# JuliaDiffusionBayes/DiffusionMCMCTools.jl

Measured on NVIDIA B200. Metric: guided path updates/sec (chains x EM steps/s, FP64), higher is better.
Workload: dtype f64

## Files before the change

diffusionmcmctools.jl_b200/csrc/dmt_api.cu:

```cuda
#include "../../include/dmt.h"
#include "kernels.cuh"
#include "fwd_kernel.cuh"
#include "sweep_kernel.cuh"
#include "sweep_ws_kernel.cuh"
#include "sweep_sp_kernel.cuh"
#include "tsit5_kernel.cuh"
#include "moments_kernel.cuh"

#include <algorithm>
#include <atomic>
#include <nvtx3/nvToolsExt.h>
#include <cmath>
#include <cstdio>
#include <cstring>
#include <dlfcn.h>
#include <stdexcept>
#include <string>
#include <unordered_map>
#include <vector>

using namespace dmt;

#ifdef DMT_ONLY_MODEL
#define DMT_FOR_MODELS(X) X(DMT_ONLY_MODEL)
#else
#define DMT_FOR_MODELS(X) X(M_FHN) X(M_LV) X(M_LORENZ) X(M_PROK) X(M_JR) X(M_OU2)
#endif

namespace {

struct DmtError : std::runtime_error {
    int code;
    DmtError(int c, const std::string &m) : std::runtime_error(m), code(c) {}
};

#define CK(call)                                                                                                   \
    do {                                                                                                           \
        cudaError_t e_ = (call);                                                                                   \
        if (e_ != cudaSuccess)                                                                                     \
            throw DmtError(DMT_ERR_CUDA, std::string(#call) + ": " + cudaGetErrorString(e_));                      \
    } while (0)
#define REQUIRE(cond, code, msg)                                                                                   \
    do {                                                                                                           \
        if (!(cond)) throw DmtError(code, msg);                                                                    \
    } while (0)

std::string g_create_error;
std::atomic<unsigned long long> g_launches{0};

struct ModelDims { int D, DW, NPAR; bool constdiff; };
bool model_dims(int model, ModelDims &md) {
    switch (model) {
    case M_FHN: md = {Model<M_FHN>::D, Model<M_FHN>::DW, Model<M_FHN>::NPAR, Model<M_FHN>::CONSTDIFF}; return true;
    case M_LV: md = {Model<M_LV>::D, Model<M_LV>::DW, Model<M_LV>::NPAR, Model<M_LV>::CONSTDIFF}; return true;
    case M_LORENZ: md = {Model<M_LORENZ>::D, Model<M_LORENZ>::DW, Model<M_LORENZ>::NPAR, Model<M_LORENZ>::CONSTDIFF}; return true;
    case M_PROK: md = {Model<M_PROK>::D, Model<M_PROK>::DW, Model<M_PROK>::NPAR, Model<M_PROK>::CONSTDIFF}; return true;
    case M_JR: md = {Model<M_JR>::D, Model<M_JR>::DW, Model<M_JR>::NPAR, Model<M_JR>::CONSTDIFF}; return true;
    case M_OU2: md = {Model<M_OU2>::D, Model<M_OU2>::DW, Model<M_OU2>::NPAR, Model<M_OU2>::CONSTDIFF}; return true;
    }
    return false;
}

template <class T> struct DevBuf {
    T *p = nullptr;
    size_t n = 0;
    void alloc(size_t count, bool zero = true) {
        release();
        n = count;
        if (count) {
            CK(cudaMalloc(&p, count * sizeof(T)));
            if (zero) {
                CK(cudaMemsetAsync(p, 0, count * sizeof(T), cudaStreamLegacy));
                CK(cudaStreamSynchronize(cudaStreamLegacy));
            }
        }
    }
    void release() {
        if (p) cudaFree(p);
        p = nullptr;
        n = 0;
    }
    ~DevBuf() { release(); }
    DevBuf() = default;
    DevBuf(const DevBuf &) = delete;
    DevBuf &operator=(const DevBuf &) = delete;
    DevBuf(DevBuf &&o) noexcept : p(o.p), n(o.n) { o.p = nullptr; o.n = 0; }
};

struct Layout {
    bool set = false;
    int nb = 0;
    std::vector<int> i0, i1;
    std::vector<uint8_t> last;
    DevBuf<int> d_i0, d_i1;
    DevBuf<uint8_t> d_last, d_ok, d_last_acc, d_acc_hist;
    DevBuf<double> d_rho, d_ll, d_ll_hist;
    LayoutDev dev{};
    bool cache_enabled = false, cache_valid = false;
    bool F_stale = false;
    DevBuf<double> d_Gl[2], d_c0l[2], d_FP[2], d_cq, d_vlast;
    DevBuf<int> d_blk_of_k;
};

struct NcclApi {
    void *h = nullptr;
    int (*GetUniqueId)(void *) = nullptr;
    int (*CommInitRank)(void **, int, struct UidByValue, int) = nullptr;
    int (*AllReduce)(const void *, void *, size_t, int, int, void *, cudaStream_t) = nullptr;
    int (*CommDestroy)(void *) = nullptr;
    const char *(*GetErrorString)(int) = nullptr;
};
struct UidByValue { char internal[128]; };
NcclApi g_nccl;
void load_nccl() {
    if (g_nccl.h) return;
    const char *names[] = {"libnccl.so.2", "libnccl.so"};
    for (const char *nm : names) {
        g_nccl.h = dlopen(nm, RTLD_NOW | RTLD_GLOBAL);
        if (g_nccl.h) break;
    }
    REQUIRE(g_nccl.h, DMT_ERR_NCCL, std::string("dlopen(libnccl.so.2) failed: ") + dlerror());
    g_nccl.GetUniqueId = (int (*)(void *))dlsym(g_nccl.h, "ncclGetUniqueId");
    g_nccl.CommInitRank = (int (*)(void **, int, UidByValue, int))dlsym(g_nccl.h, "ncclCommInitRank");
    g_nccl.AllReduce = (int (*)(const void *, void *, size_t, int, int, void *, cudaStream_t))dlsym(g_nccl.h, "ncclAllReduce");
    g_nccl.CommDestroy = (int (*)(void *))dlsym(g_nccl.h, "ncclCommDestroy");
    g_nccl.GetErrorString = (const char *(*)(int))dlsym(g_nccl.h, "ncclGetErrorString");
    REQUIRE(g_nccl.GetUniqueId && g_nccl.CommInitRank && g_nccl.AllReduce && g_nccl.CommDestroy, DMT_ERR_NCCL, "NCCL symbols missing");
}
#define NCK(call)                                                                                                  \
    do {                                                                                                           \
        int r_ = (call);                                                                                           \
        if (r_ != 0)                                                                                               \
            throw DmtError(DMT_ERR_NCCL, std::string(#call) + ": " + (g_nccl.GetErrorString ? g_nccl.GetErrorString(r_) : "nccl error")); \
    } while (0)

}

struct dmt_ctx {
    dmt_config cfg{};
    ModelDims md{};
    int D = 0, DW = 0, NPAR = 0, NH = 0, NG = 0, NAUX = 0, NOBS = 0;
    int K = 0, M = 0, P = 0, m = 0, NT = 0, NTb = 0, S = 0, NP = 0;
    std::vector<int> nsteps, tile0, step0, pt0, ppb_tile0;
    cudaStream_t stream = nullptr;
    DevCtx dev{};
    std::vector<Layout> layouts;
    std::string err;
    DevBuf<int> d_tile0, d_step0, d_pt0, d_nsteps, d_ppb_tile0, d_pset, d_k_of_tile, d_k_of_ppbtile;
    DevBuf<double> d_dt, d_sqdt, d_X, d_W, d_X0;
    DevBuf<uint8_t> d_parX, d_parW, d_parP[2];
    DevBuf<double> d_G[2][2], d_c0[2][2], d_theta[2][2], d_aux[2][2], d_obs[2], d_vart[2];
    DevBuf<double> d_scratch, d_partial, d_stats;
    DevBuf<uint8_t> d_mask;
    DevBuf<int> d_flag;
    void *nccl_comm = nullptr;
    P2PBuf *p2p_local = nullptr;
    P2PArgs p2p{};
    bool p2p_ready = false;
    int n_ranks = 1;
    int fwd_lanes = 0;
    int bwd_solver = 0;
    double bwd_reltol = 1e-3, bwd_abstol = 1e-6;
    DevBuf<int> d_steps;
    int bwd_mode = 0;
    DevBuf<double> d_xbar[2];
    std::vector<char> xbar_set[2];
    cudaStream_t copy_stream = nullptr;
    cudaEvent_t ev_gathered = nullptr, ev_copied = nullptr, ev_hist = nullptr;
    DevBuf<double> d_snap;
    DevBuf<int> d_snap_sel;
    bool pipe_ok = false;
    int sweep_mode = 0;
    std::unordered_map<const void *, size_t> resident;
    bool lazy_W = false;
    char last_fwd_kernel[96] = "";
    int W_stale_layout = -1;
    int G_owner = -1;
    bool parP_mixed = false;
    bool aux_all_linearised = true;
    DevBuf<double> d_pm_mean, d_pm_m2;
    uint64_t pm_count = 0;
    DevBuf<int> d_pm_cs, d_pm_chains;

    double *scratch(size_t n) {
        if (d_scratch.n < n) d_scratch.alloc(n, false);
        return d_scratch.p;
    }
};

namespace {

Layout &layout_of(dmt_ctx *c, int id) {
    REQUIRE(id >= 0 && id < (int)c->layouts.size(), DMT_ERR_ARG, "layout index out of range");
    REQUIRE(c->layouts[id].set, DMT_ERR_STATE, "layout not registered (dmt_set_blocks)");
    return c->layouts[id];
}

void check_side(dmt_ctx *c, int side) {
    REQUIRE(side == 0 || side == 1, DMT_ERR_ARG, "side must be 0 (accepted) or 1 (proposal)");
}
void check_law_side(dmt_ctx *c, int side) {
    check_side(c, side);
    REQUIRE(side == 0 || c->cfg.two_sided_laws, DMT_ERR_STATE, "proposal laws not allocated (dmt_config.two_sided_laws = 0)");
}
void check_range(dmt_ctx *c, int k0, int k1) { REQUIRE(0 <= k0 && k0 <= k1 && k1 < c->K, DMT_ERR_ARG, "interval range out of bounds"); }

dim3 chain_grid(dmt_ctx *c, int ny, int tpb) { return dim3((c->M + tpb - 1) / tpb, ny, 1); }
dim3 pset_grid(dmt_ctx *c, int ny, int tpb, int nz = 1) { return dim3((c->P + tpb - 1) / tpb, ny, nz); }

template <class Kernel> size_t resident_ctas(dmt_ctx *c, Kernel *kernel, int threads, size_t smem) {
    const auto it = c->resident.find((const void *)kernel);
    if (it != c->resident.end()) return it->second;
    int per_sm = 0, sms = 0;
    CK(cudaFuncSetAttribute(kernel, cudaFuncAttributeMaxDynamicSharedMemorySize, (int)smem));
    CK(cudaOccupancyMaxActiveBlocksPerMultiprocessor(&per_sm, kernel, threads, smem));
    CK(cudaDeviceGetAttribute(&sms, cudaDevAttrMultiProcessorCount, c->cfg.device));
    return c->resident[(const void *)kernel] = (size_t)per_sm * sms;
}

template <int OP> constexpr bool fwd_coop() { return OP == OP_DRAW || OP == OP_INIT || OP == OP_SWEEP; }
template <class MD> constexpr int fwd_tpb() { return MD::D >= 6 ? 32 : FWD_TPB; }
template <class MD, int OP, int G> size_t fwd_wave_threads(dmt_ctx *c) {
    return resident_ctas(c, fwd_kernel<MD, OP, fwd_tpb<MD>(), G>, fwd_tpb<MD>(), 0) * fwd_tpb<MD>();
}
template <class MD, int OP, int G> void launch_fwd_g(dmt_ctx *c, Layout &L, const FwdArgs &fa) {
    constexpr int TPB = fwd_tpb<MD>();
    fwd_wave_threads<MD, OP, G>(c);
    const dim3 grid((unsigned)(((size_t)c->M * G + TPB - 1) / TPB), L.nb, 1);
    snprintf(c->last_fwd_kernel, sizeof(c->last_fwd_kernel), "fwd_kernel<op=%d, lanes=%d%s>", OP, G, (OP == OP_SWEEP && fa.lazy_w) ? ", lazy" : "");
    ++g_launches, fwd_kernel<MD, OP, TPB, G><<<grid, TPB, 0, c->stream>>>(c->dev, L.dev, fa);
}
template <class MD, int OP> void launch_fwd_tile(dmt_ctx *c, Layout &L, const FwdArgs &fa, int lanes) {
    if constexpr (fwd_coop<OP>()) {
        if (lanes == 8) return launch_fwd_g<MD, OP, 8>(c, L, fa);
        if (lanes == 4) return launch_fwd_g<MD, OP, 4>(c, L, fa);
        if (lanes == 2) return launch_fwd_g<MD, OP, 2>(c, L, fa);
    }
    launch_fwd_g<MD, OP, 1>(c, L, fa);
}
template <class MD, int OP> int tile_lanes(dmt_ctx *c, const Layout &L) {
    if constexpr (fwd_coop<OP>()) {
        if (c->fwd_lanes) return c->fwd_lanes;
        if (MD::DW < 2) return 1;
        const size_t units = (size_t)c->M * L.nb;
        if (OP != OP_SWEEP) {
            if (units * 8 <= fwd_wave_threads<MD, OP, 8>(c)) return 8;
            if (units * 4 <= fwd_wave_threads<MD, OP, 4>(c)) return 4;
        }
        if (units * 2 <= fwd_wave_threads<MD, OP, 2>(c)) return 2;
    }
    return 1;
}

void ensure_guiding(dmt_ctx *c, Layout &L);
void ensure_W(dmt_ctx *c);
bool covers_all_intervals(dmt_ctx *c, const Layout &L) {
    std::vector<char> seen(c->K, 0);
    for (int b = 0; b < L.nb; b++)
        for (int k = L.i0[b]; k <= L.i1[b]; k++) seen[k] = 1;
    return std::all_of(seen.begin(), seen.end(), [](char s) { return s != 0; });
}

template <class MD, bool LAZY> void launch_sweep_pipe(dmt_ctx *c, Layout &L, const FwdArgs &fa) {
    constexpr size_t smem = sweep_pipe_smem<MD>();
    resident_ctas(c, sweep_pipe_kernel<MD, LAZY>, 32, smem);
    const dim3 grid((unsigned)((c->M + 31) / 32), L.nb, 1);
    snprintf(c->last_fwd_kernel, sizeof(c->last_fwd_kernel), "sweep_pipe_kernel<lanes=1%s>", LAZY ? ", lazy" : "");
    ++g_launches, sweep_pipe_kernel<MD, LAZY><<<grid, 32, smem, c->stream>>>(c->dev, L.dev, fa);
}
template <class MD> using WsWide = WsShape<6, (MD::D <= 3 ? 8 : MD::D == 4 ? 6 : 3), (MD::D <= 3 ? 4 : MD::D == 4 ? 3 : 2)>;
template <class MD, bool LAZY> size_t ws_resident_ctas(dmt_ctx *c) {
    constexpr size_t smem = sweep_ws_smem<MD, WsWide<MD>>();
    static_assert(smem <= 227 * 1024, "the rings of the warp-specialised sweep must fit one SM's shared memory");
    return resident_ctas(c, sweep_ws_kernel<MD, LAZY, WsWide<MD>>, WsWide<MD>::THREADS, smem);
}
template <class MD, bool LAZY> void launch_sweep_ws(dmt_ctx *c, Layout &L, const FwdArgs &fa) {
    using SH = WsWide<MD>;
    ws_resident_ctas<MD, LAZY>(c);
    const dim3 grid((unsigned)((c->M + 31) / 32), L.nb, 1);
    snprintf(c->last_fwd_kernel, sizeof(c->last_fwd_kernel), "sweep_ws_kernel<wide, %s>", LAZY ? "lazy" : "eager");
    ++g_launches, sweep_ws_kernel<MD, LAZY, SH><<<grid, SH::THREADS, sweep_ws_smem<MD, SH>(), c->stream>>>(c->dev, L.dev, fa);
}
template <class MD, bool LAZY> void launch_sweep_sp(dmt_ctx *c, Layout &L, const FwdArgs &fa) {
    const dim3 grid((unsigned)((c->M + 7) / 8), L.nb, 1);
    snprintf(c->last_fwd_kernel, sizeof(c->last_fwd_kernel), "sweep_sp_kernel<step lanes=4%s>", LAZY ? ", lazy" : "");
    ++g_launches, sweep_sp_kernel<MD, LAZY><<<grid, 32, 0, c->stream>>>(c->dev, L.dev, fa);
}

struct SweepChoice {
    enum Kernel { TILE, PIPE, WS, SP } kernel;
    int lanes;
    bool lazy;
};
template <class MD> SweepChoice pick_sweep(dmt_ctx *c, const Layout &L, const FwdArgs &fa) {
    const bool lazy = c->lazy_W && !fa.Z && covers_all_intervals(c, L);
    const bool eligible = c->pipe_ok && !c->parP_mixed && !fa.Z && fa.skip == 0;
    const int mode = c->sweep_mode;
    if (mode >= 2) {
        REQUIRE(eligible, DMT_ERR_UNSUPPORTED, "pipelined sweep needs one parameter set per chain in chain order, uniform law parity and device RNG");
        if (mode == 3) return {SweepChoice::WS, 1, lazy};
        if (mode == 5) return {SweepChoice::SP, 1, lazy};
        REQUIRE(c->fwd_lanes <= 1, DMT_ERR_UNSUPPORTED, "the pipelined sweep maps one lane to a (chain, block)");
        return {SweepChoice::PIPE, 1, lazy};
    }
    const SweepChoice tile{SweepChoice::TILE, tile_lanes<MD, OP_SWEEP>(c, L), lazy};
    if (mode == 1 || !eligible || c->fwd_lanes) return tile;
    const size_t ws_units = (size_t)((c->M + 31) / 32) * L.nb;
    if (ws_units <= (lazy ? ws_resident_ctas<MD, true>(c) : ws_resident_ctas<MD, false>(c))) return {SweepChoice::WS, 1, lazy};
    if (MD::DW >= 2 && (size_t)c->M * L.nb <= 14080) return {SweepChoice::SP, 1, lazy};
    if (tile.lanes == 2 || !lazy) return tile;
    return {SweepChoice::PIPE, 1, lazy};
}

template <class MD, int OP> void launch_fwd_model(dmt_ctx *c, Layout &L, FwdArgs fa) {
    if constexpr (OP == OP_SWEEP) {
        const SweepChoice s = pick_sweep<MD>(c, L, fa);
        fa.lazy_w = s.lazy;
        switch (s.kernel) {
        case SweepChoice::TILE: launch_fwd_tile<MD, OP>(c, L, fa, s.lanes); break;
        case SweepChoice::PIPE: s.lazy ? launch_sweep_pipe<MD, true>(c, L, fa) : launch_sweep_pipe<MD, false>(c, L, fa); break;
        case SweepChoice::WS: s.lazy ? launch_sweep_ws<MD, true>(c, L, fa) : launch_sweep_ws<MD, false>(c, L, fa); break;
        case SweepChoice::SP: s.lazy ? launch_sweep_sp<MD, true>(c, L, fa) : launch_sweep_sp<MD, false>(c, L, fa); break;
        }
        if (s.lazy) c->W_stale_layout = L.dev.id;
    } else {
        launch_fwd_tile<MD, OP>(c, L, fa, tile_lanes<MD, OP>(c, L));
    }
}

template <int OP> void launch_fwd(dmt_ctx *c, Layout &L, const FwdArgs &fa) {
    if (c->W_stale_layout >= 0 && OP != OP_LOGLIK) {
        const bool rewrites_all = (OP == OP_INIT) || ((OP == OP_INVSOLVE || OP == OP_INVSOLVE_LL || OP == OP_SWEEP) && covers_all_intervals(c, L));
        if (rewrites_all) c->W_stale_layout = -1;
        else ensure_W(c);
    }
    ensure_guiding(c, L);
#define DMT_CASE(MID)                                                                                              \
    case MID: launch_fwd_model<Model<MID>, OP>(c, L, fa); break;
    switch (c->cfg.model) {
        DMT_FOR_MODELS(DMT_CASE)
        default: throw DmtError(DMT_ERR_UNSUPPORTED, "model not compiled into this build of libdmt");
    }
#undef DMT_CASE
    CK(cudaGetLastError());
}

template <class MD> void launch_bwd_model(dmt_ctx *c, Layout &L, const BwdArgs &ba) {
    const int nz = c->cfg.two_sided_laws ? 2 : 1;
    if (c->bwd_solver == 1) {
        REQUIRE(!ba.use_override, DMT_ERR_UNSUPPORTED, "the guiding cache needs the RK4 backward filter (its F is affine in v only there)");
        if (c->d_steps.n < 2) c->d_steps.alloc(2);
// ... 482 lines not shown
        dim3 grid = pset_grid(ctx, k1 - k0 + 1, 128);
#define DMT_CASE(MID)                                                                                              \
    case MID: ++g_launches, aux_linearise_kernel<Model<MID>><<<grid, 128, 0, ctx->stream>>>(ctx->dev, side, store, k0, k1, tmp); break;
        switch (ctx->cfg.model) {
            DMT_FOR_MODELS(DMT_CASE)
        default: throw DmtError(DMT_ERR_UNSUPPORTED, "model not compiled into this build of libdmt");
        }
#undef DMT_CASE
        CK(cudaGetLastError());
        CK(cudaStreamSynchronize(ctx->stream));
    });
}

int32_t dmt_set_obs(dmt_ctx *ctx, int32_t side, int32_t k0, int32_t k1, const double *L, const double *Sigma, const double *v) {
    return guarded(ctx, [&] {
        check_law_side(ctx, side); check_range(ctx, k0, k1);
        if (side == 0) { ensure_W(ctx); invalidate_caches(ctx); }
        REQUIRE(L && Sigma && v, DMT_ERR_ARG, "null observation array");
        const int m = ctx->m, D = ctx->D;
        double *r0 = ctx->d_obs[0].p, *r1 = ctx->d_obs[1].p;
        put_record(ctx, side, 0, r0, r1, ctx->NOBS, 0, m * D, k0, k1, L, false);
        put_record(ctx, side, 0, r0, r1, ctx->NOBS, m * D, m * m, k0, k1, Sigma, false);
        put_record(ctx, side, 0, r0, r1, ctx->NOBS, m * D + m * m, m, k0, k1, v, false);
    });
}

int32_t dmt_equalize_laws(dmt_ctx *ctx, int32_t store_mask, int32_t k0, int32_t k1, int32_t *changed) {
    return guarded(ctx, [&] {
        check_law_side(ctx, 1); check_range(ctx, k0, k1);
        dim3 grid = pset_grid(ctx, k1 - k0 + 1, 128);
        if (ctx->d_flag.n < 1) ctx->d_flag.alloc(1);
        CK(cudaMemsetAsync(ctx->d_flag.p, 0, sizeof(int), ctx->stream));
        for (int st = 0; st < 2; st++) {
            if (!((store_mask >> st) & 1)) continue;
            ++g_launches, copy_record_kernel<<<grid, 128, 0, ctx->stream>>>(ctx->dev, st, ctx->d_theta[0][st].p, ctx->d_theta[1][st].p, ctx->NPAR, k0, k1, ctx->d_flag.p);
            ++g_launches, copy_record_kernel<<<grid, 128, 0, ctx->stream>>>(ctx->dev, st, ctx->d_aux[0][st].p, ctx->d_aux[1][st].p, ctx->NAUX, k0, k1, ctx->d_flag.p);
            if (st == 0) ++g_launches, copy_record_kernel<<<grid, 128, 0, ctx->stream>>>(ctx->dev, 0, ctx->d_obs[0].p, ctx->d_obs[1].p, ctx->NOBS, k0, k1, ctx->d_flag.p);
        }
        CK(cudaGetLastError());
        if (changed) {
            int h = 0;
            CK(cudaMemcpyAsync(&h, ctx->d_flag.p, sizeof(int), cudaMemcpyDeviceToHost, ctx->stream));
            CK(cudaStreamSynchronize(ctx->stream));
            *changed = h;
        }
    });
}

int32_t dmt_set_blocks(dmt_ctx *ctx, int32_t layout, int32_t n_blocks, const int32_t *i0, const int32_t *i1, const double *rho,
                       const uint8_t *last, int32_t ll_hist_len) {
    return guarded(ctx, [&] {
        REQUIRE(layout >= 0 && layout < (int)ctx->layouts.size(), DMT_ERR_ARG, "layout index out of range");
        REQUIRE(n_blocks >= 1 && n_blocks <= 64 && i0 && i1 && rho, DMT_ERR_ARG, "need 1 <= n_blocks <= 64 and non-null ranges/rho");
        Layout &L = ctx->layouts[layout];
        std::vector<uint8_t> lst(n_blocks);
        for (int b = 0; b < n_blocks; b++) {
            lst[b] = last ? (last[b] ? 1 : 0) : (b == n_blocks - 1 ? 1 : 0);
            REQUIRE(0 <= i0[b] && i0[b] <= i1[b] && i1[b] < ctx->K, DMT_ERR_ARG, "block range out of bounds");
            REQUIRE(lst[b] || i1[b] > i0[b], DMT_ERR_ARG, "a non-terminal block must span at least 2 intervals");
            REQUIRE(lst[b] || ctx->P == ctx->M, DMT_ERR_UNSUPPORTED,
                    "blocking freezes a per-recording artificial observation: needs n_psets == n_chains");
            REQUIRE(std::abs(rho[b]) <= 1.0, DMT_ERR_ARG, "rho must be in [-1, 1]");
        }
        const size_t M = ctx->M;
        L.nb = n_blocks;
        L.i0.assign(i0, i0 + n_blocks); L.i1.assign(i1, i1 + n_blocks); L.last = lst;
        L.d_i0.alloc(n_blocks); L.d_i1.alloc(n_blocks); L.d_last.alloc(n_blocks); L.d_rho.alloc(n_blocks);
        L.d_ll.alloc(2 * n_blocks * M); L.d_ok.alloc(n_blocks * M); L.d_last_acc.alloc(n_blocks * M);
        CK(cudaMemcpy(L.d_i0.p, i0, sizeof(int) * n_blocks, cudaMemcpyHostToDevice));
        CK(cudaMemcpy(L.d_i1.p, i1, sizeof(int) * n_blocks, cudaMemcpyHostToDevice));
        CK(cudaMemcpy(L.d_last.p, lst.data(), n_blocks, cudaMemcpyHostToDevice));
        CK(cudaMemcpy(L.d_rho.p, rho, sizeof(double) * n_blocks, cudaMemcpyHostToDevice));
        {
            std::vector<double> ninf(2 * n_blocks * M, -INFINITY);
            CK(cudaMemcpy(L.d_ll.p, ninf.data(), sizeof(double) * ninf.size(), cudaMemcpyHostToDevice));
        }
        const int hl_req = ll_hist_len >= 0 ? ll_hist_len : ctx->cfg.ll_hist_len;
        const size_t hl = hl_req > 0 ? hl_req : 0;
        if (hl) { L.d_acc_hist.alloc(hl * n_blocks * M); L.d_ll_hist.alloc(hl * 2 * n_blocks * M); }
        L.dev.nb = n_blocks; L.dev.id = layout;
        L.dev.i0 = L.d_i0.p; L.dev.i1 = L.d_i1.p; L.dev.last = L.d_last.p; L.dev.rho = L.d_rho.p;
        L.dev.ll = L.d_ll.p; L.dev.ok = L.d_ok.p; L.dev.last_acc = L.d_last_acc.p;
        L.dev.acc_hist = hl ? L.d_acc_hist.p : nullptr; L.dev.ll_hist = hl ? L.d_ll_hist.p : nullptr; L.dev.hist_len = (int)hl;
        L.set = true;
        L.cache_enabled = false; L.cache_valid = false;
        cache_set_private(L, false);
        rebuild_ppb_store(ctx);
    });
}

int32_t dmt_set_rho(dmt_ctx *ctx, int32_t layout, const double *rho) {
    return guarded(ctx, [&] {
        Layout &L = layout_of(ctx, layout);
        REQUIRE(rho, DMT_ERR_ARG, "null rho");
        CK(cudaMemcpyAsync(L.d_rho.p, rho, sizeof(double) * L.nb, cudaMemcpyHostToDevice, ctx->stream));
        CK(cudaStreamSynchronize(ctx->stream));
    });
}

int32_t dmt_set_start(dmt_ctx *ctx, const double *x0) {
    return guarded(ctx, [&] {
        REQUIRE(x0, DMT_ERR_ARG, "null x0");
        const size_t n = (size_t)ctx->D * ctx->M;
        for (int s = 0; s < 2; s++)
            CK(cudaMemcpyAsync(ctx->d_X0.p + s * ctx->dev.X0buf, x0, n * sizeof(double), cudaMemcpyHostToDevice, ctx->stream));
        CK(cudaStreamSynchronize(ctx->stream));
    });
}

static void xfer_paths(dmt_ctx *ctx, int side, double *host, bool is_x, bool upload) {
    check_side(ctx, side);
    REQUIRE(host, DMT_ERR_ARG, "null host array");
    if (!is_x) {
        if (upload && side == 0) ctx->W_stale_layout = -1;
        else ensure_W(ctx);
    }
    const size_t n = is_x ? (size_t)ctx->NP * ctx->D * ctx->M : (size_t)ctx->S * ctx->DW * ctx->M;
    DevBuf<double> nat;
    nat.alloc(n, false);
    if (upload) CK(cudaMemcpyAsync(nat.p, host, n * sizeof(double), cudaMemcpyHostToDevice, ctx->stream));
    dim3 grid = chain_grid(ctx, ctx->K, 128);
    if (is_x) ++g_launches, xfer_X_kernel<<<grid, 128, 0, ctx->stream>>>(ctx->dev, side, ctx->D, nat.p, upload ? 1 : 0);
    else ++g_launches, xfer_W_kernel<<<grid, 128, 0, ctx->stream>>>(ctx->dev, side, ctx->DW, nat.p, upload ? 1 : 0);
    CK(cudaGetLastError());
    if (!upload) CK(cudaMemcpyAsync(host, nat.p, n * sizeof(double), cudaMemcpyDeviceToHost, ctx->stream));
    CK(cudaStreamSynchronize(ctx->stream));
}
int32_t dmt_set_X(dmt_ctx *ctx, int32_t side, const double *X) { return guarded(ctx, [&] { xfer_paths(ctx, side, (double *)X, true, true); }); }
int32_t dmt_get_X(dmt_ctx *ctx, int32_t side, double *X) { return guarded(ctx, [&] { xfer_paths(ctx, side, X, true, false); }); }
int32_t dmt_set_W(dmt_ctx *ctx, int32_t side, const double *W) { return guarded(ctx, [&] { xfer_paths(ctx, side, (double *)W, false, true); }); }
int32_t dmt_get_W(dmt_ctx *ctx, int32_t side, double *W) { return guarded(ctx, [&] { xfer_paths(ctx, side, W, false, false); }); }

int32_t dmt_snapshot_paths_async(dmt_ctx *ctx, int32_t side, int32_t n_sel, const int32_t *chains, double *host_out) {
    return guarded(ctx, [&] {
        check_side(ctx, side);
        REQUIRE(n_sel >= 1 && chains && host_out, DMT_ERR_ARG, "bad snapshot arguments");
        for (int i = 0; i < n_sel; i++) REQUIRE(chains[i] >= 0 && chains[i] < ctx->M, DMT_ERR_ARG, "chain index out of range");
        if (!ctx->copy_stream) {
            CK(cudaStreamCreateWithFlags(&ctx->copy_stream, cudaStreamNonBlocking));
            CK(cudaEventCreateWithFlags(&ctx->ev_gathered, cudaEventDisableTiming));
            CK(cudaEventCreateWithFlags(&ctx->ev_copied, cudaEventDisableTiming));
            CK(cudaEventRecord(ctx->ev_copied, ctx->copy_stream));
        }
        const size_t n = (size_t)ctx->NP * ctx->D * n_sel;
        CK(cudaStreamWaitEvent(ctx->stream, ctx->ev_copied, 0));
        if (ctx->d_snap.n < n) { CK(cudaStreamSynchronize(ctx->copy_stream)); ctx->d_snap.alloc(n, false); }
        if (ctx->d_snap_sel.n < (size_t)n_sel) { CK(cudaStreamSynchronize(ctx->copy_stream)); ctx->d_snap_sel.alloc(n_sel, false); }
        CK(cudaMemcpyAsync(ctx->d_snap_sel.p, chains, sizeof(int) * n_sel, cudaMemcpyHostToDevice, ctx->stream));
        ++g_launches, gather_X_kernel<<<dim3((n_sel + 63) / 64, ctx->K), 64, 0, ctx->stream>>>(ctx->dev, side, ctx->D, ctx->d_snap_sel.p, n_sel, ctx->d_snap.p);
        CK(cudaGetLastError());
        CK(cudaEventRecord(ctx->ev_gathered, ctx->stream));
        CK(cudaStreamWaitEvent(ctx->copy_stream, ctx->ev_gathered, 0));
        CK(cudaMemcpyAsync(host_out, ctx->d_snap.p, n * sizeof(double), cudaMemcpyDeviceToHost, ctx->copy_stream));
        CK(cudaEventRecord(ctx->ev_copied, ctx->copy_stream));
    });
}
static void get_paths_of(dmt_ctx *ctx, int side, int n_sel, const int32_t *chains, double *out, bool is_x) {
    check_side(ctx, side);
    if (!is_x) ensure_W(ctx);
    REQUIRE(n_sel >= 1 && chains && out, DMT_ERR_ARG, "bad chain selection");
    for (int i = 0; i < n_sel; i++) REQUIRE(chains[i] >= 0 && chains[i] < ctx->M, DMT_ERR_ARG, "chain index out of range");
    const size_t n = (is_x ? (size_t)ctx->NP * ctx->D : (size_t)ctx->S * ctx->DW) * n_sel;
    DevBuf<double> d;
    DevBuf<int> sel;
    d.alloc(n, false);
    sel.alloc(n_sel, false);
// ... 682 lines not shown
```

diffusionmcmctools.jl_b200/csrc/sweep_kernel.cuh:

```cuda
#pragma once
#include "fwd_kernel.cuh"
#include <type_traits>

namespace dmt {

template <int N, int I = 0, class F> __device__ __forceinline__ void static_for(F &&f) {
    if constexpr (I < N) {
        f(std::integral_constant<int, I>{});
        static_for<N, I + 1>(f);
    }
}

__device__ __forceinline__ bool elect_one_lane() {
    uint32_t pred;
    asm volatile("{\n.reg .pred p;\nelect.sync _|p, 0xffffffff;\nselp.u32 %0, 1, 0, p;\n}" : "=r"(pred));
    return pred != 0;
}
template <class MD> constexpr int sweep_pipe_minb() { return MD::D <= 3 ? 10 : 1; }

template <class MD> constexpr size_t sweep_pipe_smem() {
    constexpr int D = MD::D, NG = D * (D + 1) / 2 + D;
    return (size_t)2 * (NG * 128 + 8) * 8 + (size_t)(D * D + D) * 32 * 8 + 2 * 8;
}

template <class MD, bool LAZYW>
__global__ void __launch_bounds__(32, sweep_pipe_minb<MD>()) sweep_pipe_kernel(const DevCtx cx, const LayoutDev ly, const FwdArgs fa) {
    constexpr int D = MD::D, DW = MD::DW, NPAR = MD::NPAR, NH = D * (D + 1) / 2, NG = NH + D, NAUX = D * D + D + NH;
    constexpr int STAGE = NG * 128 + 8;
    extern __shared__ __align__(128) unsigned char sw_smem[];
    double *ring = reinterpret_cast<double *>(sw_smem);
    double *cst = ring + 2 * STAGE;
    uint64_t *bars = reinterpret_cast<uint64_t *>(cst + (D * D + D) * 32);

    const int lane = threadIdx.x;
    const int c0 = blockIdx.x * 32, b = blockIdx.y;
    if (c0 >= cx.M) return;
    const int c_raw = c0 + lane;
    const int c = min(c_raw, cx.M - 1);
    const bool live = c_raw < cx.M;
    const size_t M = cx.M, P = cx.P;
    const int ps = c;
    const int i0 = ly.i0[b], i1 = ly.i1[b];
    const bool last = ly.last[b] != 0;
    const double rho = ly.rho[b], crho = sqrt(1.0 - rho * rho);
    const uint32_t chunk_bytes = 32u * (uint32_t)min(32, cx.M - c0);
    const size_t gstr = P * 4;

    if (lane == 0) { mbar_init(&bars[0], 1); mbar_init(&bars[1], 1); }
    asm volatile("fence.mbarrier_init.release.cluster;" ::: "memory");
    __syncwarp();

    int kn = i0, qn = 0, ntl_n = (cx.nsteps[i0] + 3) >> 2, t0_n = cx.tile0[i0], n_prod = 0;
    const double *gp_n = g_tile_of<NG>(cx, ly, i0, i1, last, 0, c0).base;
    const double *xin_n = cx.X + (size_t)cx.parX[(size_t)i0 * M + c] * cx.Xbuf + ((size_t)t0_n * D * M + c) * 4;
    bool more = true;
    double xnx[D][4];
    auto prefetch = [&]() {
        if (!more) return;
        if (elect_one_lane()) {
            uint64_t *bar = &bars[n_prod & 1];
            double *dst = ring + (size_t)(n_prod & 1) * STAGE;
            mbar_expect_tx(bar, NG * chunk_bytes + 64u);
#pragma unroll
            for (int a = 0; a < NG; a++) bulk_g2s(dst + a * 128, gp_n + ((size_t)qn * NG + a) * gstr, chunk_bytes, bar);
            bulk_g2s(dst + NG * 128, cx.dt + (size_t)(t0_n + qn) * 4, 32u, bar);
            bulk_g2s(dst + NG * 128 + 4, cx.sqdt + (size_t)(t0_n + qn) * 4, 32u, bar);
        }
#pragma unroll
        for (int i = 0; i < D; i++) ld256(xin_n + ((size_t)qn * D + i) * M * 4, xnx[i]);
        n_prod++;
        if (++qn == ntl_n) {
            qn = 0;
            if (++kn <= i1) {
                ntl_n = (cx.nsteps[kn] + 3) >> 2;
                t0_n = cx.tile0[kn];
                gp_n = g_tile_of<NG>(cx, ly, kn, i1, last, 0, c0).base;
                xin_n = cx.X + (size_t)cx.parX[(size_t)kn * M + c] * cx.Xbuf + ((size_t)t0_n * D * M + c) * 4;
            } else more = false;
        }
    };
    prefetch();

    double x[D], xo[D];
    {
        const int sl = cx.parX[(size_t)i0 * M + c];
#pragma unroll
        for (int i = 0; i < D; i++) { x[i] = cx.X0[sl * cx.X0buf + ((size_t)i0 * D + i) * M + c]; xo[i] = x[i]; }
    }
    double ll = 0.0, llo = 0.0;
    bool ok = true;
    int n_cons = 0;

    for (int k = i0; k <= i1; ++k) {
        const GTile<NG> gt = g_tile_of<NG>(cx, ly, k, i1, last, 0, ps);
        double th[NPAR];
        {
            const double *tp = cx.theta[gt.slot][gt.store] + (size_t)k * NPAR * P + ps;
#pragma unroll
            for (int i = 0; i < NPAR; i++) th[i] = tp[(size_t)i * P];
        }
        const typename MD::Par par(th);
        {
            const double *ap = cx.aux[gt.slot][gt.store] + (size_t)k * NAUX * P + ps;
#pragma unroll
            for (int i = 0; i < D * D + D; i++) cst[i * 32 + lane] = ap[(size_t)i * P];
        }
        double at[NH];
        if (!MD::CONSTDIFF) {
            const double *ap = cx.aux[gt.slot][gt.store] + (size_t)k * NAUX * P + ps;
#pragma unroll
            for (int i = 0; i < NH; i++) at[i] = ap[(size_t)(D * D + D + i) * P];
        }
        const int nst = cx.nsteps[k], t0 = cx.tile0[k];
        const uint8_t pw = cx.parW[(size_t)k * M + c], px = cx.parX[(size_t)k * M + c];
        double *Wacc = cx.W + (size_t)pw * cx.Wbuf + ((size_t)t0 * DW * M + c) * 4;
        double *Wprop = cx.W + (size_t)(1 ^ pw) * cx.Wbuf + ((size_t)t0 * DW * M + c) * 4;
        double *Xout = cx.X + (size_t)(1 ^ px) * cx.Xbuf + ((size_t)t0 * D * M + c) * 4;
        if (k > i0) {
#pragma unroll
            for (int i = 0; i < D; i++) x[i] = cx.X0[(size_t)px * cx.X0buf + ((size_t)k * D + i) * M + c];
        }
        if (live) {
            double *x0p = cx.X0 + (size_t)(1 ^ px) * cx.X0buf + (size_t)k * D * M + c;
#pragma unroll
            for (int i = 0; i < D; i++) x0p[(size_t)i * M] = xo[i];
        }
        const int ntl = (nst + 3) >> 2;
        for (int q = 0; q < ntl; ++q) {
            double xt[D][4];
#pragma unroll
            for (int i = 0; i < D; i++)
#pragma unroll
                for (int s = 0; s < 4; s++) xt[i][s] = xnx[i][s];
            prefetch();
            if (q == ntl - 1 && k < i1) {
                const int k1 = k + 1;
                const int store1 = (k1 == i1 && !last) ? 1 : 0;
                const int slot1 = cx.parP[store1][(size_t)k1 * P + ps];
                const double *tp = cx.theta[slot1][store1] + (size_t)k1 * NPAR * P + ps;
#pragma unroll
                for (int i = 0; i < NPAR; i++) prefetch_l2(tp + (size_t)i * P);
                const double *ap = cx.aux[slot1][store1] + (size_t)k1 * NAUX * P + ps;
#pragma unroll
                for (int i = 0; i < (MD::CONSTDIFF ? D * D + D : NAUX); i++) prefetch_l2(ap + (size_t)i * P);
#pragma unroll
                for (int i = 0; i < D; i++) {
                    prefetch_l2(cx.X0 + ((size_t)k1 * D + i) * M + c);
                    prefetch_l2(cx.X0 + cx.X0buf + ((size_t)k1 * D + i) * M + c);
                }
                prefetch_l2(cx.parX + (size_t)k1 * M + c);
                prefetch_l2(cx.parW + (size_t)k1 * M + c);
            }
            double z[4 * DW];
            tile_normals<DW>(cx.seed, cx.chain_offset + (uint32_t)c, (uint32_t)(t0 + q), fa.iter, (uint32_t)ly.id, z);

            mbar_wait(&bars[n_cons & 1], (uint32_t)(n_cons >> 1) & 1u);
            const double *st = ring + (size_t)(n_cons & 1) * STAGE;
            const double *sg = st + lane * 4;
            n_cons++;
            if (k == i0 && q == 0) {
                double s0 = -*gt.c0;
#pragma unroll
                for (int i = 0; i < D; i++) {
                    double hx = 0.0;
#pragma unroll
                    for (int j = 0; j < D; j++) hx = fma(sg[sidx<D>(i, j) * 128], x[j], hx);
                    s0 += x[i] * (sg[(NH + i) * 128] - 0.5 * hx);
                }
                ll = s0;
                llo = s0;
            }
            double w[LAZYW ? 1 : DW][4], wo[LAZYW ? 1 : DW][4], xot[D][4];
            auto step = [&](auto s_c, auto full_c) {
                constexpr int s = decltype(s_c)::value;
                constexpr bool FULL = decltype(full_c)::value;
                const int i = 4 * q + s;
                if (FULL || i < nst) {
                    double Hs[NH], F[D], Bm[D * D], beta[D], gd[D], G = 0.0;
#pragma unroll
                    for (int a = 0; a < NH; a++) Hs[a] = sg[a * 128 + s];
#pragma unroll
                    for (int a = 0; a < D; a++) F[a] = sg[(NH + a) * 128 + s];
#pragma unroll
                    for (int a = 0; a < D * D; a++) Bm[a] = cst[a * 32 + lane];
#pragma unroll
                    for (int a = 0; a < D; a++) beta[a] = cst[(D * D + a) * 32 + lane];
                    const double dt = st[NG * 128 + s], sq = st[NG * 128 + 4 + s];
                    const typename MD::Diff df(par, x);
                    guided_terms<MD, true>(par, df, Bm, beta, at, Hs, F, x, gd, G);
                    ll = fma(G, dt, ll);
                    double xn[D], res[D], dwv[DW];
#pragma unroll
                    for (int a = 0; a < D; a++) xn[a] = xt[a][s];
#pragma unroll
                    for (int a = 0; a < D; a++) res[a] = xn[a] - x[a] - gd[a] * dt;
                    df.inv_sig(res, dwv);
#pragma unroll
                    for (int a = 0; a < D; a++) x[a] = xn[a];
                    double dwo[DW];
                    static_for<DW>([&](auto j_c) {
                        constexpr int j = decltype(j_c)::value;
                        const double xi = z[s * DW + j];
                        dwo[j] = rho * dwv[j] + crho * sq * xi;
                        if (!LAZYW) { w[j][s] = dwv[j]; wo[j][s] = dwo[j]; }
                    });
                    if (FULL || ok) {
                        double swo[D], gdo[D], Go = 0.0, xon[D];
                        const typename MD::Diff dfo(par, xo);
                        guided_terms<MD, true>(par, dfo, Bm, beta, at, Hs, F, xo, gdo, Go);
                        llo = fma(Go, dt, llo);
                        dfo.sig_mul(dwo, swo);
#pragma unroll
                        for (int a = 0; a < D; a++) xon[a] = fma(gdo[a], dt, xo[a]) + swo[a];
                        bool fin = dfo.ok();
#pragma unroll
                        for (int a = 0; a < D; a++) fin = fin && isfinite(xon[a]);
                        ok = ok && fin && MD::bound_ok(par, xon);
#pragma unroll
                        for (int a = 0; a < D; a++) { xot[a][s] = xon[a]; xo[a] = xon[a]; }
                    } else {
#pragma unroll
                        for (int a = 0; a < D; a++) xot[a][s] = 0.0;
                    }
                } else {
#pragma unroll
                    for (int a = 0; a < D; a++) xot[a][s] = 0.0;
                    if (!LAZYW) {
#pragma unroll
                        for (int j = 0; j < DW; j++) { w[j][s] = 0.0; wo[j][s] = 0.0; }
                    }
                }
            };
            if (4 * q + 4 <= nst) static_for<4>([&](auto s_c) { step(s_c, std::true_type{}); });
            else static_for<4>([&](auto s_c) { step(s_c, std::false_type{}); });
            if (live) {
                if (!LAZYW) {
#pragma unroll
                    for (int j = 0; j < DW; j++) st256(Wacc + ((size_t)q * DW + j) * M * 4, w[j]);
#pragma unroll
                    for (int j = 0; j < DW; j++) st256(Wprop + ((size_t)q * DW + j) * M * 4, wo[j]);
                }
#pragma unroll
                for (int i = 0; i < D; i++) st256(Xout + ((size_t)q * D + i) * M * 4, xot[i]);
            }
            __syncwarp();
        }
    }
    if (live) {
        ly.ll[(size_t)b * M + c] = ll;
        ly.ll[((size_t)ly.nb + b) * M + c] = ok ? llo : -INFINITY;
        ly.ok[(size_t)b * M + c] = ok ? 1 : 0;
    }
}

}
```

Measured before the change: 22.71 billion.

## Add persistent ticket-scheduled sweep pipeline kernel with cross-interval state handoff

Turns the sweep pipeline kernel into an optional persistent kernel. Warps pull (block, interval, chain-group) tasks from an atomic ticket counter, working through a precomputed task list in interval-depth order. Per-chain state (xo, ll, llo, ok) is handed between consecutive intervals through a global buffer, with release/acquire flags and spin-waits so a later interval waits for the earlier one. The kernel can also pack several warps per CTA for low-dimensional models. The aim is to balance load across uneven block lengths and fill the SMs, at the cost of a memset, atomics, spin latency, and extra global traffic for the handoff.

```diff
diff --git a/diffusionmcmctools.jl_b200/csrc/dmt_api.cu b/diffusionmcmctools.jl_b200/csrc/dmt_api.cu
--- a/diffusionmcmctools.jl_b200/csrc/dmt_api.cu
+++ b/diffusionmcmctools.jl_b200/csrc/dmt_api.cu
@@ -100,6 +100,9 @@
     bool F_stale = false;
     DevBuf<double> d_Gl[2], d_c0l[2], d_FP[2], d_cq, d_vlast;
     DevBuf<int> d_blk_of_k;
+    DevBuf<int> d_task;
+    DevBuf<unsigned> d_ticket;
+    DevBuf<double> d_hand;
 };
 
 struct NcclApi {
@@ -172,6 +175,7 @@
     bool pipe_ok = false;
     int sweep_mode = 0;
     std::unordered_map<const void *, size_t> resident;
+    int n_sm = 0;
     bool lazy_W = false;
     char last_fwd_kernel[96] = "";
     int W_stale_layout = -1;
@@ -211,11 +215,11 @@
 template <class Kernel> size_t resident_ctas(dmt_ctx *c, Kernel *kernel, int threads, size_t smem) {
     const auto it = c->resident.find((const void *)kernel);
     if (it != c->resident.end()) return it->second;
-    int per_sm = 0, sms = 0;
+    int per_sm = 0;
     CK(cudaFuncSetAttribute(kernel, cudaFuncAttributeMaxDynamicSharedMemorySize, (int)smem));
     CK(cudaOccupancyMaxActiveBlocksPerMultiprocessor(&per_sm, kernel, threads, smem));
-    CK(cudaDeviceGetAttribute(&sms, cudaDevAttrMultiProcessorCount, c->cfg.device));
-    return c->resident[(const void *)kernel] = (size_t)per_sm * sms;
+    if (!c->n_sm) CK(cudaDeviceGetAttribute(&c->n_sm, cudaDevAttrMultiProcessorCount, c->cfg.device));
+    return c->resident[(const void *)kernel] = (size_t)per_sm * c->n_sm;
 }
 
 template <int OP> constexpr bool fwd_coop() { return OP == OP_DRAW || OP == OP_INIT || OP == OP_SWEEP; }
@@ -263,10 +267,22 @@
 
 template <class MD, bool LAZY> void launch_sweep_pipe(dmt_ctx *c, Layout &L, const FwdArgs &fa) {
     constexpr size_t smem = sweep_pipe_smem<MD>();
-    resident_ctas(c, sweep_pipe_kernel<MD, LAZY>, 32, smem);
-    const dim3 grid((unsigned)((c->M + 31) / 32), L.nb, 1);
+    constexpr int WPC = MD::D <= 3 ? 4 : 1;
+    const size_t groups = (c->M + 31) / 32, units = groups * L.nb;
+    const size_t warps = resident_ctas(c, sweep_pipe_kernel<MD, LAZY, WPC>, 32 * WPC, WPC * smem) * WPC;
+    const size_t S = (size_t)c->n_sm * 4;
+    const size_t n = std::min(warps, units >= 2 * S ? 2 * S : (units >= S && units * 100 < S * 123) ? S : 0);
     snprintf(c->last_fwd_kernel, sizeof(c->last_fwd_kernel), "sweep_pipe_kernel<lanes=1%s>", LAZY ? ", lazy" : "");
-    ++g_launches, sweep_pipe_kernel<MD, LAZY><<<grid, 32, smem, c->stream>>>(c->dev, L.dev, fa);
+    if (n < S) {
+        resident_ctas(c, sweep_pipe_kernel<MD, LAZY, 1>, 32, smem);
+        ++g_launches, sweep_pipe_kernel<MD, LAZY, 1><<<dim3((unsigned)groups, L.nb, 1), 32, smem, c->stream>>>(c->dev, L.dev, fa, PipeSched{});
+        return;
+    }
+    if (L.d_ticket.n != 1 + units) L.d_ticket.alloc(1 + units, false);
+    if (L.d_hand.n != (size_t)(MD::D + 3) * units * 32) L.d_hand.alloc((size_t)(MD::D + 3) * units * 32, false);
+    CK(cudaMemsetAsync(L.d_ticket.p, 0, sizeof(unsigned) * (1 + units), c->stream));
+    const PipeSched sc{L.d_task.p, (int)(L.d_task.n * groups), L.d_ticket.p, L.d_hand.p};
+    ++g_launches, sweep_pipe_kernel<MD, LAZY, WPC><<<(unsigned)(n / WPC), 32 * WPC, WPC * smem, c->stream>>>(c->dev, L.dev, fa, sc);
 }
 template <class MD> using WsWide = WsShape<6, (MD::D <= 3 ? 8 : MD::D == 4 ? 6 : 3), (MD::D <= 3 ? 4 : MD::D == 4 ? 3 : 2)>;
 template <class MD, bool LAZY> size_t ws_resident_ctas(dmt_ctx *c) {
@@ -915,6 +931,17 @@
         L.dev.i0 = L.d_i0.p; L.dev.i1 = L.d_i1.p; L.dev.last = L.d_last.p; L.dev.rho = L.d_rho.p;
         L.dev.ll = L.d_ll.p; L.dev.ok = L.d_ok.p; L.dev.last_acc = L.d_last_acc.p;
         L.dev.acc_hist = hl ? L.d_acc_hist.p : nullptr; L.dev.ll_hist = hl ? L.d_ll_hist.p : nullptr; L.dev.hist_len = (int)hl;
+        {
+            std::vector<int> task;
+            for (int j = 0;; j++) {
+                const size_t n0 = task.size();
+                for (int b = 0; b < n_blocks; b++)
+                    if (i0[b] + j <= i1[b]) task.push_back(b + 64 * j);
+                if (task.size() == n0) break;
+            }
+            L.d_task.alloc(task.size(), false);
+            CK(cudaMemcpy(L.d_task.p, task.data(), sizeof(int) * task.size(), cudaMemcpyHostToDevice));
+        }
         L.set = true;
         L.cache_enabled = false; L.cache_valid = false;
         cache_set_private(L, false);
diff --git a/diffusionmcmctools.jl_b200/csrc/sweep_kernel.cuh b/diffusionmcmctools.jl_b200/csrc/sweep_kernel.cuh
--- a/diffusionmcmctools.jl_b200/csrc/sweep_kernel.cuh
+++ b/diffusionmcmctools.jl_b200/csrc/sweep_kernel.cuh
@@ -18,80 +18,110 @@
 }
 template <class MD> constexpr int sweep_pipe_minb() { return MD::D <= 3 ? 10 : 1; }
 
-template <class MD> constexpr size_t sweep_pipe_smem() {
+template <class MD> __host__ __device__ constexpr size_t sweep_pipe_smem() {
     constexpr int D = MD::D, NG = D * (D + 1) / 2 + D;
-    return (size_t)2 * (NG * 128 + 8) * 8 + (size_t)(D * D + D) * 32 * 8 + 2 * 8;
-}
-
-template <class MD, bool LAZYW>
-__global__ void __launch_bounds__(32, sweep_pipe_minb<MD>()) sweep_pipe_kernel(const DevCtx cx, const LayoutDev ly, const FwdArgs fa) {
+    return ((size_t)2 * (NG * 128 + 8) * 8 + (size_t)(D * D + D) * 32 * 8 + 2 * 8 + 127) / 128 * 128;
+}
+
+struct PipeSched {
+    const int *task;
+    int n_tasks;
+    unsigned *ticket;
+    double *hand;
+};
+
+__device__ __forceinline__ unsigned ld_acquire_gpu(const unsigned *p) {
+    unsigned v;
+    asm volatile("ld.acquire.gpu.global.u32 %0, [%1];" : "=r"(v) : "l"(p) : "memory");
+    return v;
+}
+__device__ __forceinline__ void st_release_gpu(unsigned *p, unsigned v) { asm volatile("st.release.gpu.global.u32 [%0], %1;" ::"l"(p), "r"(v) : "memory"); }
+
+template <class MD, bool LAZYW, int WPC>
+__global__ void __launch_bounds__(32 * WPC, WPC == 1 ? sweep_pipe_minb<MD>() : 2)
+    sweep_pipe_kernel(const DevCtx cx, const LayoutDev ly, const FwdArgs fa, const PipeSched sc) {
     constexpr int D = MD::D, DW = MD::DW, NPAR = MD::NPAR, NH = D * (D + 1) / 2, NG = NH + D, NAUX = D * D + D + NH;
     constexpr int STAGE = NG * 128 + 8;
     extern __shared__ __align__(128) unsigned char sw_smem[];
-    double *ring = reinterpret_cast<double *>(sw_smem);
+    const int lane = threadIdx.x & 31;
+    double *ring = reinterpret_cast<double *>(sw_smem + (threadIdx.x >> 5) * sweep_pipe_smem<MD>());
     double *cst = ring + 2 * STAGE;
     uint64_t *bars = reinterpret_cast<uint64_t *>(cst + (D * D + D) * 32);
-
-    const int lane = threadIdx.x;
-    const int c0 = blockIdx.x * 32, b = blockIdx.y;
-    if (c0 >= cx.M) return;
-    const int c_raw = c0 + lane;
-    const int c = min(c_raw, cx.M - 1);
-    const bool live = c_raw < cx.M;
     const size_t M = cx.M, P = cx.P;
-    const int ps = c;
-    const int i0 = ly.i0[b], i1 = ly.i1[b];
-    const bool last = ly.last[b] != 0;
-    const double rho = ly.rho[b], crho = sqrt(1.0 - rho * rho);
-    const uint32_t chunk_bytes = 32u * (uint32_t)min(32, cx.M - c0);
+    const int G = (cx.M + 31) >> 5;
     const size_t gstr = P * 4;
+    const bool tickets = sc.task != nullptr;
 
     if (lane == 0) { mbar_init(&bars[0], 1); mbar_init(&bars[1], 1); }
     asm volatile("fence.mbarrier_init.release.cluster;" ::: "memory");
     __syncwarp();
 
-    int kn = i0, qn = 0, ntl_n = (cx.nsteps[i0] + 3) >> 2, t0_n = cx.tile0[i0], n_prod = 0;
-    const double *gp_n = g_tile_of<NG>(cx, ly, i0, i1, last, 0, c0).base;
-    const double *xin_n = cx.X + (size_t)cx.parX[(size_t)i0 * M + c] * cx.Xbuf + ((size_t)t0_n * D * M + c) * 4;
+    int un, kn;
     bool more = true;
+    auto take_ticket = [&]() {
+        unsigned t = 0;
+        if (lane == 0) t = atomicAdd(sc.ticket, 1u);
+        t = __shfl_sync(0xffffffffu, t, 0);
+        if (t >= (unsigned)sc.n_tasks) { more = false; return; }
+        const int e = (int)(t / (unsigned)G), en = sc.task[e], bn = en & 63;
+        un = bn * G + (int)(t - (unsigned)e * G);
+        kn = ly.i0[bn] + (en >> 6);
+    };
+    if (tickets) take_ticket();
+    else {
+        un = blockIdx.y * G + blockIdx.x;
+        kn = ly.i0[blockIdx.y];
+    }
+    int qn = 0, ntl_n = 0, t0_n = 0, n_prod = 0, tu[2] = {0, 0}, tk[2] = {0, 0};
+    uint32_t chunk_n = 0;
+    const double *gp_n = nullptr, *xin_n = nullptr;
+    auto start_cursor = [&]() {
+        const int bn = un / G, c0n = (un - bn * G) * 32, cn = min(c0n + lane, cx.M - 1);
+        ntl_n = (cx.nsteps[kn] + 3) >> 2;
+        t0_n = cx.tile0[kn];
+        chunk_n = 32u * (uint32_t)min(32, cx.M - c0n);
+        gp_n = g_tile_of<NG>(cx, ly, kn, ly.i1[bn], ly.last[bn] != 0, 0, c0n).base;
+        xin_n = cx.X + (size_t)cx.parX[(size_t)kn * M + cn] * cx.Xbuf + ((size_t)t0_n * D * M + cn) * 4;
+    };
+    if (more) start_cursor();
     double xnx[D][4];
     auto prefetch = [&]() {
         if (!more) return;
         if (elect_one_lane()) {
             uint64_t *bar = &bars[n_prod & 1];
             double *dst = ring + (size_t)(n_prod & 1) * STAGE;
-            mbar_expect_tx(bar, NG * chunk_bytes + 64u);
-#pragma unroll
-            for (int a = 0; a < NG; a++) bulk_g2s(dst + a * 128, gp_n + ((size_t)qn * NG + a) * gstr, chunk_bytes, bar);
+            mbar_expect_tx(bar, NG * chunk_n + 64u);
+#pragma unroll
+            for (int a = 0; a < NG; a++) bulk_g2s(dst + a * 128, gp_n + ((size_t)qn * NG + a) * gstr, chunk_n, bar);
             bulk_g2s(dst + NG * 128, cx.dt + (size_t)(t0_n + qn) * 4, 32u, bar);
             bulk_g2s(dst + NG * 128 + 4, cx.sqdt + (size_t)(t0_n + qn) * 4, 32u, bar);
         }
 #pragma unroll
         for (int i = 0; i < D; i++) ld256(xin_n + ((size_t)qn * D + i) * M * 4, xnx[i]);
+        if (n_prod & 1) { tu[1] = un; tk[1] = kn; } else { tu[0] = un; tk[0] = kn; }
         n_prod++;
         if (++qn == ntl_n) {
             qn = 0;
-            if (++kn <= i1) {
-                ntl_n = (cx.nsteps[kn] + 3) >> 2;
-                t0_n = cx.tile0[kn];
-                gp_n = g_tile_of<NG>(cx, ly, kn, i1, last, 0, c0).base;
-                xin_n = cx.X + (size_t)cx.parX[(size_t)kn * M + c] * cx.Xbuf + ((size_t)t0_n * D * M + c) * 4;
-            } else more = false;
+            if (tickets) take_ticket();
+            else if (++kn > ly.i1[blockIdx.y]) more = false;
+            if (more) start_cursor();
         }
     };
     prefetch();
 
-    double x[D], xo[D];
-    {
-        const int sl = cx.parX[(size_t)i0 * M + c];
-#pragma unroll
-        for (int i = 0; i < D; i++) { x[i] = cx.X0[sl * cx.X0buf + ((size_t)i0 * D + i) * M + c]; xo[i] = x[i]; }
-    }
-    double ll = 0.0, llo = 0.0;
+    double xo[D], ll = 0.0, llo = 0.0;
     bool ok = true;
     int n_cons = 0;
-
-    for (int k = i0; k <= i1; ++k) {
+    while (n_cons < n_prod) {
+        const int u = (n_cons & 1) ? tu[1] : tu[0], k = (n_cons & 1) ? tk[1] : tk[0];
+        const int b = u / G, c0 = (u - b * G) * 32;
+        const int c_raw = c0 + lane;
+        const int c = min(c_raw, cx.M - 1);
+        const bool live = c_raw < cx.M;
+        const int ps = c;
+        const int i0 = ly.i0[b], i1 = ly.i1[b];
+        const bool last = ly.last[b] != 0;
+        const double rho = ly.rho[b], crho = sqrt(1.0 - rho * rho);
         const GTile<NG> gt = g_tile_of<NG>(cx, ly, k, i1, last, 0, ps);
         double th[NPAR];
         {
@@ -116,14 +146,13 @@
         double *Wacc = cx.W + (size_t)pw * cx.Wbuf + ((size_t)t0 * DW * M + c) * 4;
         double *Wprop = cx.W + (size_t)(1 ^ pw) * cx.Wbuf + ((size_t)t0 * DW * M + c) * 4;
         double *Xout = cx.X + (size_t)(1 ^ px) * cx.Xbuf + ((size_t)t0 * D * M + c) * 4;
-        if (k > i0) {
-#pragma unroll
-            for (int i = 0; i < D; i++) x[i] = cx.X0[(size_t)px * cx.X0buf + ((size_t)k * D + i) * M + c];
-        }
-        if (live) {
-            double *x0p = cx.X0 + (size_t)(1 ^ px) * cx.X0buf + (size_t)k * D * M + c;
-#pragma unroll
-            for (int i = 0; i < D; i++) x0p[(size_t)i * M] = xo[i];
+        double x[D];
+#pragma unroll
+        for (int i = 0; i < D; i++) x[i] = cx.X0[(size_t)px * cx.X0buf + ((size_t)k * D + i) * M + c];
+        if (k == i0) {
+#pragma unroll
+            for (int i = 0; i < D; i++) xo[i] = x[i];
+            ok = true;
         }
         const int ntl = (nst + 3) >> 2;
         for (int q = 0; q < ntl; ++q) {
@@ -133,26 +162,46 @@
 #pragma unroll
                 for (int s = 0; s < 4; s++) xt[i][s] = xnx[i][s];
             prefetch();
-            if (q == ntl - 1 && k < i1) {
-                const int k1 = k + 1;
-                const int store1 = (k1 == i1 && !last) ? 1 : 0;
-                const int slot1 = cx.parP[store1][(size_t)k1 * P + ps];
-                const double *tp = cx.theta[slot1][store1] + (size_t)k1 * NPAR * P + ps;
+            if (q == ntl - 1 && n_prod == n_cons + 2) {
+                const int u1 = (n_prod & 1) ? tu[0] : tu[1], k1 = (n_prod & 1) ? tk[0] : tk[1];
+                const int b1 = u1 / G, c1 = min((u1 - b1 * G) * 32 + lane, cx.M - 1), ps1 = c1;
+                const int store1 = (k1 == ly.i1[b1] && !ly.last[b1]) ? 1 : 0;
+                const int slot1 = cx.parP[store1][(size_t)k1 * P + ps1];
+                const double *tp = cx.theta[slot1][store1] + (size_t)k1 * NPAR * P + ps1;
 #pragma unroll
                 for (int i = 0; i < NPAR; i++) prefetch_l2(tp + (size_t)i * P);
-                const double *ap = cx.aux[slot1][store1] + (size_t)k1 * NAUX * P + ps;
+                const double *ap = cx.aux[slot1][store1] + (size_t)k1 * NAUX * P + ps1;
 #pragma unroll
                 for (int i = 0; i < (MD::CONSTDIFF ? D * D + D : NAUX); i++) prefetch_l2(ap + (size_t)i * P);
 #pragma unroll
                 for (int i = 0; i < D; i++) {
-                    prefetch_l2(cx.X0 + ((size_t)k1 * D + i) * M + c);
-                    prefetch_l2(cx.X0 + cx.X0buf + ((size_t)k1 * D + i) * M + c);
-                }
-                prefetch_l2(cx.parX + (size_t)k1 * M + c);
-                prefetch_l2(cx.parW + (size_t)k1 * M + c);
+                    prefetch_l2(cx.X0 + ((size_t)k1 * D + i) * M + c1);
+                    prefetch_l2(cx.X0 + cx.X0buf + ((size_t)k1 * D + i) * M + c1);
+                }
+                prefetch_l2(cx.parX + (size_t)k1 * M + c1);
+                prefetch_l2(cx.parW + (size_t)k1 * M + c1);
             }
             double z[4 * DW];
             tile_normals<DW>(cx.seed, cx.chain_offset + (uint32_t)c, (uint32_t)(t0 + q), fa.iter, (uint32_t)ly.id, z);
+            if (q == 0) {
+                if (tickets && k > i0) {
+                    const unsigned *done = sc.ticket + 1 + u;
+                    while (ld_acquire_gpu(done) < (unsigned)(k - i0)) __nanosleep(100);
+                    const double *h = sc.hand + (size_t)u * 32 + lane;
+                    const size_t hs = (size_t)G * ly.nb * 32;
+#pragma unroll
+                    for (int i = 0; i < D; i++) xo[i] = __ldcg(h + i * hs);
+                    ll = __ldcg(h + D * hs);
+                    llo = __ldcg(h + (D + 1) * hs);
+                    ok = __ldcg(h + (D + 2) * hs) != 0.0;
+                    __syncwarp();
+                }
+                if (live) {
+                    double *x0p = cx.X0 + (size_t)(1 ^ px) * cx.X0buf + (size_t)k * D * M + c;
+#pragma unroll
+                    for (int i = 0; i < D; i++) x0p[(size_t)i * M] = xo[i];
+                }
+            }
 
             mbar_wait(&bars[n_cons & 1], (uint32_t)(n_cons >> 1) & 1u);
             const double *st = ring + (size_t)(n_cons & 1) * STAGE;
@@ -245,12 +294,24 @@
             }
             __syncwarp();
         }
+        if (k == i1) {
+            if (live) {
+                ly.ll[(size_t)b * M + c] = ll;
+                ly.ll[((size_t)ly.nb + b) * M + c] = ok ? llo : -INFINITY;
+                ly.ok[(size_t)b * M + c] = ok ? 1 : 0;
+            }
+        } else if (tickets) {
+            double *h = sc.hand + (size_t)u * 32 + lane;
+            const size_t hs = (size_t)G * ly.nb * 32;
+#pragma unroll
+            for (int i = 0; i < D; i++) __stcg(h + i * hs, xo[i]);
+            __stcg(h + D * hs, ll);
+            __stcg(h + (D + 1) * hs, llo);
+            __stcg(h + (D + 2) * hs, ok ? 1.0 : 0.0);
+            __syncwarp();
+            if (lane == 0) st_release_gpu(sc.ticket + 1 + u, (unsigned)(k - i0 + 1));
+        }
     }
-    if (live) {
-        ly.ll[(size_t)b * M + c] = ll;
-        ly.ll[((size_t)ly.nb + b) * M + c] = ok ? llo : -INFINITY;
-        ly.ok[(size_t)b * M + c] = ok ? 1 : 0;
-    }
-}
-
-}
+}
+
+}
```

Result: faster. 23.97 billion, median of 6 (+5.6%).
